# heliaxdev/ark-plonk

Measured on AMD Instinct MI355X. Metric: proofs/sec at 2^20 constraints (BLS12-381, KZG10); MSM G1-adds/s, higher is better.
Workload: dtype u32 limbs (256/384-bit Montgomery integers)

## Files before the change

### ark_plonk_amd/build.py

```python
from __future__ import annotations

import os
import subprocess
import sys
from concurrent.futures import ThreadPoolExecutor

HERE = os.path.dirname(os.path.abspath(__file__))
CSRC = os.path.join(HERE, "csrc")
OBJ = os.path.join(CSRC, "obj")
LIB = os.path.join(HERE, "libark_plonk_amd.so")
HIPCC = os.environ.get("HIPCC", "/opt/rocm/bin/hipcc")
FLAGS = ["--offload-arch=gfx950", "-O3", "-std=c++17", "-fPIC", "-Wall", "-Wno-unused-function", "-Wno-unused-variable",
         "-mllvm", "-pragma-unroll-threshold=1000000", "-Wpass-failed"]

FIELD_HDRS = ["field_common.cuh", "field.cuh", "fieldu.cuh", "fields.cuh", "curve_params.h", "zk_common.h"]
HOST_HDRS = FIELD_HDRS + ["ecu.cuh", "ctx.h", "g1_host.h", "../../include/ark_plonk_amd.h"]
API_HDRS = HOST_HDRS + ["api_internal.h"]
FR_IO, ZBOUND, POINT_IO = ["fr_io.cuh"], ["fr_io.cuh", "zbound.cuh"], ["point_io.cuh"]
DOMAIN, DEV_SCAN = ["fr_io.cuh", "domain.cuh"], ["dev_scan.cuh"]
GADGET = ["gadget_common.cuh"]
BLOCK_INV = ["block_inverse.cuh"]
G1_LIFT = ["g1_lift.cuh"]
PAIRING = ["pairing.cuh", "pairing_params.h"]
REPLAY = ["strobe.cuh", "replay_walk.cuh"]
API_UNITS = ("api_ctx", "residency", "srs", "commit", "round", "api_host", "api_poly")
MSM_UNITS = ("msm_accumulate", "msm_reduce", "msm_sort", "msm_plan")


def jobs():
    out = [(f"{u}.o", f"{u}.hip", [], API_HDRS + (DOMAIN if u == "api_poly" else [])) for u in API_UNITS] + [
        ("hostio.o", "hostio.hip", [], HOST_HDRS),
        ("wire.o", "wire.hip", [], HOST_HDRS + REPLAY),
        ("kzg.o", "kzg.hip", [], HOST_HDRS + ZBOUND),
        ("lookup.o", "lookup.hip", [], HOST_HDRS + ZBOUND + DEV_SCAN),
        ("grand_product.o", "grand_product.hip", [], HOST_HDRS + DOMAIN),
        ("quotient.o", "quotient.hip", [], HOST_HDRS + ZBOUND + DOMAIN),
        ("quadtest.o", "quadtest.hip", [], HOST_HDRS + ["ecq.cuh"]),
        ("ntt.o", "ntt.hip", [], HOST_HDRS + DOMAIN + ["ntt_pass.cuh"]),
        ("ntt_pass_table.o", "ntt_pass_table.hip", [], []),
        ("msm_dispatch.o", "msm_dispatch.hip", [], HOST_HDRS),
        ("ipa.o", "ipa.hip", [], API_HDRS + FR_IO + POINT_IO + BLOCK_INV),
        ("compile.o", "compile.hip", [], API_HDRS + DOMAIN + DEV_SCAN),
        ("check.o", "check.hip", [], API_HDRS + ZBOUND + DOMAIN),
        ("gadget_layout.o", "gadget_layout.hip", [], API_HDRS + FR_IO + GADGET),
        ("gadget_witness.o", "gadget_witness.hip", [], API_HDRS + FR_IO + GADGET + BLOCK_INV),
        ("lookup_map.o", "lookup_map.hip", [], API_HDRS + FR_IO),
        ("verify.o", "verify.hip", [], API_HDRS + DOMAIN + BLOCK_INV + G1_LIFT),
        ("replay.o", "replay.hip", [], API_HDRS + REPLAY),
        ("g1_segments.o", "g1_segments.hip", [], API_HDRS + BLOCK_INV),
        ("ipa_setup.o", "ipa_setup.hip", [], API_HDRS + BLOCK_INV + G1_LIFT + ["h2c.cuh"]),
        ("pairing.o", "pairing.hip", [], API_HDRS + PAIRING),
    ]
    for c in (0, 1):
        for unit in MSM_UNITS:
            out.append((f"{unit}_c{c}.o", f"{unit}.hip", [f"-DZK_CURVE_SEL={c}"] + os.environ.get("ARK_PLONK_AMD_MSM_FLAGS", "").split(),
                        HOST_HDRS + POINT_IO + ["msm_common.cuh"] + (["ecq.cuh"] if unit == "msm_reduce" else [])))
        for s in range(3, 10):
            out.append((f"ntt_pass_c{c}_s{s}.o", "ntt_pass_inst.hip", [f"-DZK_CURVE_SEL={c}", f"-DZK_NTT_S={s}"],
                        FIELD_HDRS + ["ntt_pass.cuh"]))
    return out


PMC_UNITS = {
    "pmc_msm_accumulate.json": [("msm_accumulate.hip", ["-DZK_CURVE_SEL=0"])],
    "pmc_ntt.json": [("ntt.hip", [])] + [("ntt_pass_inst.hip", ["-DZK_CURVE_SEL=0", f"-DZK_NTT_S={s}"]) for s in range(3, 10)],
}


def device_asm(src: str, defs=(), timeout: float = 900) -> str:
    import re
    cmd = [HIPCC] + FLAGS + list(defs) + ["--cuda-device-only", "-S", os.path.join(CSRC, src), "-o", "-"]
    r = subprocess.run(cmd, capture_output=True, text=True, timeout=timeout)
    if r.returncode != 0:
        raise RuntimeError("hipcc failed: " + " ".join(cmd) + "\n" + r.stderr[-4000:])
    return re.sub(r"__hip_cuid_[0-9a-f]+", "__hip_cuid_X", r.stdout)


def device_code_sha256(units, workers: int = 8) -> str:
    import hashlib
    with ThreadPoolExecutor(max_workers=workers) as ex:
        texts = list(ex.map(lambda u: device_asm(*u), units))
    return hashlib.sha256("".join(texts).encode()).hexdigest()


def _stale(target: str, deps) -> bool:
    if not os.path.exists(target):
        return True
    t = os.path.getmtime(target)
    return any(os.path.getmtime(d) > t for d in deps)


def build(force: bool = False, verbose: bool = False, workers: int | None = None) -> str:
    os.makedirs(OBJ, exist_ok=True)
    todo = []
    objs = []
    for obj, src, defs, hdrs in jobs():
        o = os.path.join(OBJ, obj)
        objs.append(o)
        deps = [os.path.join(CSRC, src)] + [os.path.join(CSRC, h) for h in hdrs]
        if force or _stale(o, deps):
            todo.append([HIPCC] + FLAGS + defs + ["-c", os.path.join(CSRC, src), "-o", o])
    todo.sort(key=lambda c: (0 if "/msm_" in " ".join(c[-3:]) else 1, -int(next((d.split("=")[1] for d in c if d.startswith("-DZK_NTT_S=")), 0))))

    def run(cmd):
        if verbose:
            print(" ".join(cmd), flush=True)
        r = subprocess.run(cmd, capture_output=True, text=True)
        if r.returncode != 0:
            raise RuntimeError("hipcc failed: " + " ".join(cmd) + "\n" + r.stderr[-4000:])
        return r.stderr

    if todo:
        n = workers or min(len(todo), max(1, (os.cpu_count() or 4)))
        with ThreadPoolExecutor(max_workers=n) as ex:
            for err in ex.map(run, todo):
                if verbose and err.strip():
                    print(err, file=sys.stderr)
    if force or todo or _stale(LIB, objs):
        cmd = [HIPCC, "--offload-arch=gfx950", "-shared", "-fPIC", "-o", LIB] + objs
        if verbose:
            print(" ".join(cmd[:6]), "...", flush=True)
        subprocess.check_call(cmd)
    return LIB


if __name__ == "__main__":
    print(build(force="--force" in sys.argv, verbose=True))
```

### ark_plonk_amd/csrc/fieldu.cuh

```cuda
#pragma once
#include "field_common.cuh"

template <class P>
struct Fu {
    static constexpr int NL = P::NL;
    static constexpr int SAT = P::SAT_WORDS;
    static constexpr uint32_t M = (1u << 29) - 1u;
    uint32_t v[NL];

    ZK_HD static Fu zero() {
        Fu r;
#pragma unroll
        for (int i = 0; i < NL; ++i) r.v[i] = 0;
        return r;
    }
    ZK_HD static Fu one() {
        Fu r;
#pragma unroll
        for (int i = 0; i < NL; ++i) r.v[i] = P::ONE(i);
        return r;
    }
    ZK_HD bool limbs_zero() const {
        uint32_t o = 0;
#pragma unroll
// ... 89 lines not shown
    }
    ZK_HD static Fu sub_raw8(const Fu& a, const Fu& b) {
        Fu t;
#pragma unroll
        for (int i = 0; i < NL; ++i) t.v[i] = a.v[i] + P::ZB8(i) - b.v[i];
        return t;
    }
    ZK_HD static Fu sub_raw16(const Fu& a, const Fu& b) {
        Fu t;
#pragma unroll
        for (int i = 0; i < NL; ++i) t.v[i] = a.v[i] + P::ZB16(i) - b.v[i];
        return t;
    }

    ZK_HD static Fu mul(const Fu& a, const Fu& b) {
        uint32_t m[NL];
        Fu r;
        uint64_t carry = 0;
#pragma unroll
        for (int k = 0; k < NL; ++k) {
            uint64_t a0 = 0, a1 = 0, am = 0;
#pragma unroll
            for (int i = 0; i <= k; ++i) {
                if (i & 1) a1 += (uint64_t)a.v[i] * b.v[k - i];
                else a0 += (uint64_t)a.v[i] * b.v[k - i];
            }
#pragma unroll
            for (int i = 0; i < k; ++i) am += (uint64_t)m[i] * P::MOD(k - i);
            uint64_t t = a0 + a1 + am + carry;
            m[k] = ((uint32_t)t * P::PINV) & M;
            t += (uint64_t)m[k] * P::MOD(0);
            carry = t >> 29;
        }
#pragma unroll
        for (int k = NL; k < 2 * NL - 1; ++k) {
            uint64_t a0 = 0, a1 = 0, am = 0;
#pragma unroll
            for (int i = k - NL + 1; i < NL; ++i) {
                if (i & 1) a1 += (uint64_t)a.v[i] * b.v[k - i];
                else a0 += (uint64_t)a.v[i] * b.v[k - i];
                am += (uint64_t)m[i] * P::MOD(k - i);
            }
            uint64_t t = a0 + a1 + am + carry;
            r.v[k - NL] = (uint32_t)t & M;
            carry = t >> 29;
        }
        r.v[NL - 1] = (uint32_t)carry;
        return r;
    }
    ZK_HD static uint64_t fence64(uint64_t t) {
#if defined(__HIP_DEVICE_COMPILE__)
        asm("" : "+v"(t));
#endif
        return t;
    }
    ZK_HD static Fu mul_fenced(const Fu& a, const Fu& b) {
        uint32_t m[NL];
        Fu r;
        uint64_t carry = 0;
#pragma unroll
        for (int k = 0; k < NL; ++k) {
            uint64_t t = fence64(carry + (uint64_t)a.v[0] * b.v[k]);
#pragma unroll
            for (int i = 1; i <= k; ++i) t += (uint64_t)a.v[i] * b.v[k - i];
#pragma unroll
            for (int i = 0; i < k; ++i) t += (uint64_t)m[i] * P::MOD(k - i);
            m[k] = ((uint32_t)t * P::PINV) & M;
            t += (uint64_t)m[k] * P::MOD(0);
            carry = t >> 29;
        }
#pragma unroll
        for (int k = NL; k < 2 * NL - 1; ++k) {
            uint64_t t = fence64(carry + (uint64_t)a.v[k - NL + 1] * b.v[NL - 1]);
#pragma unroll
            for (int i = k - NL + 2; i < NL; ++i) t += (uint64_t)a.v[i] * b.v[k - i];
#pragma unroll
            for (int i = k - NL + 1; i < NL; ++i) t += (uint64_t)m[i] * P::MOD(k - i);
            r.v[k - NL] = (uint32_t)t & M;
            carry = t >> 29;
        }
        r.v[NL - 1] = (uint32_t)carry;
        return r;
    }
    ZK_HD static Fu sqr(const Fu& a) {
        uint32_t m[NL], a2[NL];
        Fu r;
#pragma unroll
        for (int i = 0; i < NL; ++i) a2[i] = a.v[i] << 1;
        uint64_t carry = 0;
#pragma unroll
        for (int k = 0; k < NL; ++k) {
            uint64_t aa = 0, am = 0;
#pragma unroll
            for (int i = 0; 2 * i < k; ++i) aa += (uint64_t)a2[i] * a.v[k - i];
            if ((k & 1) == 0) aa += (uint64_t)a.v[k / 2] * a.v[k / 2];
#pragma unroll
            for (int i = 0; i < k; ++i) am += (uint64_t)m[i] * P::MOD(k - i);
            uint64_t t = aa + am + carry;
            m[k] = ((uint32_t)t * P::PINV) & M;
            t += (uint64_t)m[k] * P::MOD(0);
            carry = t >> 29;
        }
#pragma unroll
        for (int k = NL; k < 2 * NL - 1; ++k) {
            uint64_t aa = 0, am = 0;
#pragma unroll
            for (int i = k - NL + 1; 2 * i < k; ++i) aa += (uint64_t)a2[i] * a.v[k - i];
            if ((k & 1) == 0) aa += (uint64_t)a.v[k / 2] * a.v[k / 2];
#pragma unroll
            for (int i = k - NL + 1; i < NL; ++i) am += (uint64_t)m[i] * P::MOD(k - i);
            uint64_t t = aa + am + carry;
            r.v[k - NL] = (uint32_t)t & M;
            carry = t >> 29;
        }
        r.v[NL - 1] = (uint32_t)carry;
        return r;
    }

    ZK_HD bool is_zero_mod_reduced() const {
        if (v[0] != 0 && v[0] != P::MOD(0)) return false;
        uint32_t dz = 0, dp = 0;
#pragma unroll
        for (int i = 0; i < NL; ++i) {
            dz |= v[i];
            dp |= v[i] ^ P::MOD(i);
        }
        return dz == 0 || dp == 0;
    }
    ZK_HD bool is_zero_mod() const { return mul(*this, one()).is_zero_mod_reduced(); }

    ZK_HD static Fu canonical_lt2p(const Fu& a) {
        Fu d;
#pragma unroll
        for (int i = 0; i < NL; ++i) d.v[i] = a.v[i] - P::MOD(i);
        normalize(d);
        const bool neg = ((int32_t)d.v[NL - 1]) < 0;
        Fu r;
#pragma unroll
        for (int i = 0; i < NL; ++i) r.v[i] = neg ? a.v[i] : d.v[i];
        return r;
    }

    ZK_HD static Fu from_sat(const uint32_t* w) {
        Fu t = split_words(w);
        Fu c;
#pragma unroll
        for (int i = 0; i < NL; ++i) c.v[i] = P::C_IN(i);
        return mul(t, c);
    }
    ZK_HD void to_sat(uint32_t* w) const {
        Fu c;
#pragma unroll
        for (int i = 0; i < NL; ++i) c.v[i] = P::C_OUT(i);
        Fu t = canonical_lt2p(mul(*this, c));
        t.pack_words(w);
    }
    ZK_HD static Fu split_words(const uint32_t* w) {
        Fu t;
#pragma unroll
        for (int i = 0; i < NL; ++i) {
            const int bit = 29 * i;
            const int wi = bit >> 5, off = bit & 31;
            uint64_t lo = wi < SAT ? w[wi] : 0u;
            uint64_t hi = (wi + 1) < SAT ? w[wi + 1] : 0u;
            t.v[i] = (uint32_t)(((hi << 32) | lo) >> off) & M;
        }
// ... 16 lines not shown
```

### ark_plonk_amd/csrc/ntt.hip

```cpp
#include "ctx.h"
#include "domain.cuh"

#include "ntt_pass.cuh"

namespace {

template <class Fr>
struct PowBits {
    Fr p[32];
};
template <class Fr>
__global__ void gen_pow_table(void* out, uint64_t n, PowBits<Fr> pb, Fr mul, int mode, uint32_t log_m, uint32_t log_mprev, Fr to_rp) {
    uint64_t i = (uint64_t)blockIdx.x * blockDim.x + threadIdx.x;
    if (i >= n) return;
    uint64_t e = i;
    if (mode == 1) {
        uint64_t col = i & ((1ull << log_m) - 1);
        uint64_t k = i >> log_m;
        e = (col * k) & ((1ull << log_mprev) - 1);
    }
    Fr r = mul;
    for (int b = 0; b < 32; ++b) {
        if ((e >> b) & 1ull) r = Fr::mul(r, pb.p[b]);
    }
    st_fr<Fr>(out, i, Fr::mul(r, to_rp));
}

template <class FU>
__global__ void split_table(const void* packed, void* out, uint64_t n) {
    const uint64_t i = (uint64_t)blockIdx.x * blockDim.x + threadIdx.x;
    if (i >= n) return;
    const FU x = ld_u<FU>(packed, i);
    uint32_t w[4 * TW_INNER_U4];
#pragma unroll
    for (int k = 0; k < 4 * TW_INNER_U4; ++k) w[k] = k < FU::NL ? x.v[k] : 0u;
    uint4* q = reinterpret_cast<uint4*>(out) + TW_INNER_U4 * i;
#pragma unroll
    for (int k = 0; k < TW_INNER_U4; ++k) q[k] = make_uint4(w[4 * k], w[4 * k + 1], w[4 * k + 2], w[4 * k + 3]);
}

template <class Fr>
__global__ void ntt_tiny(const void* in, void* out, uint64_t in_len, uint32_t log_n, Fr w , Fr pre_g ,
                         Fr post_g , Fr scale ) {
    if (threadIdx.x != 0 || blockIdx.x != 0) return;
    const uint32_t n = 1u << log_n;
    Fr x[4], y[4];
    Fr gp = Fr::one();
    for (uint32_t i = 0; i < n; ++i) {
        x[i] = i < in_len ? Fr::mul(ld_fr<Fr>(in, i), gp) : Fr::zero();
        gp = Fr::mul(gp, pre_g);
    }
    Fr wi = Fr::one(), pg = scale;
    for (uint32_t i = 0; i < n; ++i) {
        Fr acc = Fr::zero(), wij = Fr::one();
        for (uint32_t j = 0; j < n; ++j) {
            acc = Fr::add(acc, Fr::mul(x[j], wij));
            wij = Fr::mul(wij, wi);
        }
        y[i] = Fr::mul(acc, pg);
        pg = Fr::mul(pg, post_g);
        wi = Fr::mul(wi, w);
    }
    for (uint32_t i = 0; i < n; ++i) st_fr<Fr>(out, i, y[i]);
}

template <class Fr>
__global__ void fr_convert_kernel(const void* in, void* out, uint64_t n, int to_mont) {
    uint64_t i = (uint64_t)blockIdx.x * blockDim.x + threadIdx.x;
    if (i >= n) return;
    Fr x = ld_fr<Fr>(in, i);
    st_fr<Fr>(out, i, to_mont ? Fr::to_mont(x) : Fr::from_mont(x));
}
template <class Fr>
__global__ void fr_mul_kernel(const void* a, const void* b, void* out, uint64_t n) {
    uint64_t i = (uint64_t)blockIdx.x * blockDim.x + threadIdx.x;
    if (i >= n) return;
    st_fr<Fr>(out, i, Fr::mul(ld_fr<Fr>(a, i), ld_fr<Fr>(b, i)));
}

template <class Fr>
PowBits<Fr> make_powbits(Fr base) {
    PowBits<Fr> pb;
    Fr cur = base;
    for (int b = 0; b < 32; ++b) {
        pb.p[b] = cur;
        cur = Fr::sqr(cur);
    }
    return pb;
}

template <class C>
int launch_pow_table(zk_ctx* c, void* out, uint64_t n, typename C::Fr base, typename C::Fr mul, int mode, uint32_t log_m,
                     uint32_t log_mprev) {
    typedef typename C::Fr Fr;
    if (n == 0) return ZK_OK;
    PowBits<Fr> pb = make_powbits(base);
    const Fr to_rp = to_rprime(Fr::one());
    const int T = 256;
    uint64_t blocks = (n + T - 1) / T;
    hipLaunchKernelGGL(gen_pow_table<Fr>, dim3((unsigned)blocks), dim3(T), 0, c->stream, out, n, pb, mul, mode, log_m, log_mprev, to_rp);
    ZK_HIP_TRY(hipGetLastError());
    return ZK_OK;
}

bool decompose(uint32_t log_n, int forced, int& n_pass, int s[4]) {
    s[0] = s[1] = s[2] = s[3] = 0;
    if (forced == 0 && log_n <= 9) {
        n_pass = 1;
        s[0] = (int)log_n;
        return true;
    }
    n_pass = forced ? forced : (int)((log_n + 8) / 9);
    if (n_pass > 4) return true;
    int base = (int)log_n / n_pass, extra = (int)log_n % n_pass;
    for (int i = 0; i < n_pass; ++i) s[i] = base + (i < extra ? 1 : 0);
    return forced == 0 || (s[n_pass - 1] >= 3 && s[0] <= 9);
}
int forced_passes(const zk_ctx* c, uint32_t log_n) { return log_n < 3 ? 0 : c->tune.ntt_passes; }

template <class C>
int get_inner_tw(zk_ctx* c, int s, bool inverse, void** out) {
    typedef typename C::Fr Fr;
    uint64_t key = ((uint64_t)C::ID << 40) | ((uint64_t)(inverse ? 1 : 0) << 32) | (uint64_t)s;
    auto it = c->inner_tw.find(key);
    if (it != c->inner_tw.end()) {
        *out = it->second;
        return ZK_OK;
    }
    uint64_t cnt = s >= 1 ? (1ull << (s - 1)) : 1;
    void* packed = nullptr;
    void* p = nullptr;
    if (hipMalloc(&packed, cnt * sizeof(Fr)) != hipSuccess) return zk_alloc_refused();
    if (hipMalloc(&p, cnt * TW_INNER_U4 * 16) != hipSuccess) {
        (void)hipFree(packed);
        return zk_alloc_refused();
    }
    Fr w = domain_root<C>((uint32_t)s);
    if (inverse) w = Fr::inverse(w);
    int rc = launch_pow_table<C>(c, packed, cnt, w, Fr::one(), 0, 0, 0);
    if (!rc) {
        const int T = 256;
        hipLaunchKernelGGL(split_table<typename C::FrU>, dim3((unsigned)((cnt + T - 1) / T)), dim3(T), 0, c->stream, packed, p, cnt);
        if (hipGetLastError() != hipSuccess || hipStreamSynchronize(c->stream) != hipSuccess) rc = ZK_ERR_HIP;
    }
    (void)hipFree(packed);
    if (rc) {
        (void)hipFree(p);
        return rc;
    }
    c->inner_tw[key] = p;
    *out = p;
    return ZK_OK;
}

template <class C>
int get_plan(zk_ctx* c, uint32_t log_n, bool inverse, NttPlan** out) {
    typedef typename C::Fr Fr;
    const int forced = forced_passes(c, log_n);
    uint64_t key = ((uint64_t)C::ID << 40) | ((uint64_t)forced << 36) | ((uint64_t)(inverse ? 1 : 0) << 32) | log_n;
    auto it = c->plans.find(key);
    if (it != c->plans.end()) {
        *out = it->second;
        return ZK_OK;
    }
    int n_pass, s[4];
    if (!decompose(log_n, forced, n_pass, s)) return ZK_ERR_UNSUPPORTED;
    NttPlan* pl = new NttPlan();
    pl->curve = C::ID;
    pl->log_n = log_n;
    pl->inverse = inverse;
    pl->n_pass = n_pass;
    for (int i = 0; i < 4; ++i) pl->s[i] = s[i];
    uint32_t log_mprev = log_n;
    for (int p = 0; p < pl->n_pass; ++p) {
        if (log_n >= 3) {
            int rc = get_inner_tw<C>(c, pl->s[p], inverse, &pl->tw_inner[p]);
            if (rc) { delete pl; return rc; }
        }
        if (p + 1 < pl->n_pass) {
            uint32_t log_m = log_mprev - (uint32_t)pl->s[p];
            uint64_t cnt = 1ull << log_mprev;
            hipError_t e = hipMalloc(&pl->tw_pass[p], cnt * sizeof(Fr));
            if (e != hipSuccess) { delete pl; return zk_alloc_refused(); }
            Fr w = domain_root<C>(log_mprev);
            if (inverse) w = Fr::inverse(w);
            int rc = launch_pow_table<C>(c, pl->tw_pass[p], cnt, w, Fr::one(), 1, log_m, log_mprev);
            if (rc) { delete pl; return rc; }
            log_mprev = log_m;
        }
    }
    c->plans[key] = pl;
    *out = pl;
    return ZK_OK;
}

template <class C>
int ensure_coset(zk_ctx* c, bool inv, uint64_t len, void** out) {
    typedef typename C::Fr Fr;
    DevBuf& buf = inv ? c->coset_inv_pow[C::ID] : c->coset_pow[C::ID];
    size_t& have = inv ? c->coset_inv_len[C::ID] : c->coset_len[C::ID];
    if (have < len) {
        ZK_HIP_TRY(hipStreamSynchronize(c->stream));
        uint64_t want = 1;
        while (want < len) want <<= 1;
        int rc = buf.ensure(want * sizeof(Fr));
        if (rc) return rc;
        Fr g = coset_gen<C>();
        if (inv) g = Fr::inverse(g);
        rc = launch_pow_table<C>(c, buf.p, want, g, Fr::one(), 0, 0, 0);
        if (rc) return rc;
        have = want;
    }
    *out = buf.p;
    return ZK_OK;
}

typedef int (*NttPassLauncher)(int final_pass, const NttPassArgs* a, hipStream_t st);
extern "C" NttPassLauncher zk_ntt_pass_launcher(int curve, int s);

template <class C>
int dispatch_pass(zk_ctx* c, int s, bool final_pass, const NttPassArgs& a) {
    if (s < 3 || s > 9) return ZK_ERR_UNSUPPORTED;
    NttPassLauncher fn = zk_ntt_pass_launcher(C::ID, s);
    if (!fn) return ZK_ERR_UNSUPPORTED;
    hipError_t e = (hipError_t)fn(final_pass ? 1 : 0, &a, c->stream);
    ZK_HIP_TRY(e);
    return ZK_OK;
}

template <class C>
int ntt_run(zk_ctx* c, int kind, uint32_t log_n, uint32_t n_polys, const void* const* d_ins, const size_t* in_lens, void* const* d_outs) {
    typedef typename C::Fr Fr;
    if (!domain_log_ok<C>(log_n)) return ZK_ERR_DOMAIN_TOO_LARGE;
    if (n_polys == 0 || n_polys > 16) return ZK_ERR_BAD_ARG;
    const uint64_t N = 1ull << log_n;
    size_t in_len = 0;
    bool all_quarter = true;
    for (uint32_t i = 0; i < n_polys; ++i) {
        if (in_lens[i] > N) return ZK_ERR_BAD_ARG;
        if (in_lens[i] > in_len) in_len = in_lens[i];
        if ((uint64_t)in_lens[i] * 4 > N) all_quarter = false;
    }
    const void* d_in = d_ins[0];
    void* d_out = d_outs[0];
    const bool inverse = (kind == ZK_NTT_IFFT || kind == ZK_NTT_COSET_IFFT);
    int rc;
    Fr n_inv = Fr::inverse(Fr::from_u64(N));
    if (log_n < 3) {
        Fr w = domain_root<C>(log_n);
        if (inverse) w = Fr::inverse(w);
        Fr g = coset_gen<C>();
        Fr pre_g = kind == ZK_NTT_COSET_FFT ? g : Fr::one();
        Fr post_g = kind == ZK_NTT_COSET_IFFT ? Fr::inverse(g) : Fr::one();
        ProfScope ps(c, "ntt_pass");
        for (uint32_t i = 0; i < n_polys; ++i)
            hipLaunchKernelGGL(ntt_tiny<Fr>, dim3(1), dim3(64), 0, c->stream, d_ins[i], d_outs[i], (uint64_t)in_lens[i], log_n, w, pre_g, post_g,
                               inverse ? n_inv : Fr::one());
        ZK_HIP_TRY(hipGetLastError());
        return ZK_OK;
    }
    {
        int np, sp[4];
        if (!decompose(log_n, forced_passes(c, log_n), np, sp)) return ZK_ERR_UNSUPPORTED;
    }
    void* pre = nullptr;
    void* post = nullptr;
    if (kind == ZK_NTT_COSET_FFT && in_len > 0) {
        rc = ensure_coset<C>(c, false, in_len, &pre);
        if (rc) return rc;
    }
    if (kind == ZK_NTT_COSET_IFFT) {
        rc = ensure_coset<C>(c, true, N, &post);
        if (rc) return rc;
    }
    NttPlan* pl = nullptr;
    rc = get_plan<C>(c, log_n, inverse, &pl);
    if (rc) return rc;
    if (pl->n_pass > 4) return ZK_ERR_UNSUPPORTED;
    void* work = nullptr;
    if (pl->n_pass > 1) {
        rc = c->ntt_work.ensure((size_t)n_polys * N * sizeof(Fr));
        if (rc) return rc;
        work = c->ntt_work.p;
    }
    uint32_t log_mprev = log_n;
    NttPassArgs a;
    ProfScope ps(c, "ntt_pass");
    for (int p = 0; p < pl->n_pass; ++p) {
        const int s = pl->s[p];
        const bool last = (p + 1 == pl->n_pass);
        memset(&a, 0, sizeof a);
        a.log_n = log_n;
        a.in = (p == 0) ? d_in : work;
        a.out = last ? d_out : work;
        a.in_len = (p == 0) ? in_lens[0] : N;
        if (n_polys > 1) {
            a.n_batch = n_polys;
            for (uint32_t i = 0; i < n_polys; ++i) {
                void* wk = (char*)work + (size_t)i * N * sizeof(Fr);
                a.ins[i] = (p == 0) ? d_ins[i] : wk;
                a.outs[i] = last ? d_outs[i] : wk;
                a.in_lens[i] = (p == 0) ? in_lens[i] : N;
            }
        }
        a.tw_inner = pl->tw_inner[p];
        a.pre_mul = (p == 0) ? pre : nullptr;
        const uint32_t LC = 9u - (uint32_t)s;
        if (!last) {
            uint32_t log_m = log_mprev - (uint32_t)s;
            uint32_t logc = LC < log_m ? LC : log_m;
            a.logc = logc;
            a.log_m = log_m;
            a.log_mprev = log_mprev;
            a.tw_pass = pl->tw_pass[p];
            a.n_tiles = (uint32_t)(N >> ((uint32_t)s + logc));
            a.quarter = (p == 0 && s >= 3 && all_quarter) ? 1u : 0u;
            log_mprev = log_m;
        } else {
            uint32_t s1 = (pl->n_pass > 1) ? (uint32_t)pl->s[0] : 0;
            uint32_t logc = LC < s1 ? LC : s1;
            a.logc = logc;
            a.s1 = s1;
            a.s2 = pl->n_pass == 4 ? (uint32_t)pl->s[1] : 0u;
            a.post_mul = post;
            const Fr sc = to_rprime(inverse ? n_inv : Fr::one());
            for (int i = 0; i < 8; ++i) a.scale[i] = sc.v[i];
            a.n_tiles = (uint32_t)(N >> ((uint32_t)s + logc));
        }
        rc = dispatch_pass<C>(c, s, last, a);
        if (rc) return rc;
        if (c->profiling) c->prof["ntt_passes"].launches += 1;
    }
    return ZK_OK;
}

}

int ntt_run_dev(zk_ctx* c, int curve, int kind, uint32_t log_n, const void* d_in, size_t in_len, void* d_out) {
    return ntt_run_batch_dev(c, curve, kind, log_n, 1, &d_in, &in_len, &d_out);
}

int ntt_run_batch_dev(zk_ctx* c, int curve, int kind, uint32_t log_n, uint32_t n_polys, const void* const* d_ins, const size_t* in_lens,
                      void* const* d_outs) {
    if (kind < 0 || kind > 3) return ZK_ERR_BAD_ARG;
    for (uint32_t base = 0; base < n_polys; base += 16) {
        const uint32_t cnt = n_polys - base < 16 ? n_polys - base : 16;
        const int rc = zk_on_curve(curve, ZK_ERR_BAD_ARG, [&](auto cv) {
            return ntt_run<decltype(cv)>(c, kind, log_n, cnt, d_ins + base, in_lens + base, d_outs + base);
        });
        if (rc) return rc;
    }
    return ZK_OK;
}

int ntt_prepare(zk_ctx* c, int curve, uint32_t log_n) {
    NttPlan* pl;
    if (log_n < 3) return ZK_OK;
    for (int inv = 0; inv < 2; ++inv) {
        const int rc = zk_on_curve(curve, ZK_ERR_BAD_ARG, [&](auto cv) {
            typedef decltype(cv) Cv;
            if (!domain_log_ok<Cv>(log_n)) return ZK_ERR_DOMAIN_TOO_LARGE;
            return get_plan<Cv>(c, log_n, inv != 0, &pl);
        });
        if (rc) return rc;
    }
    return ZK_OK;
}

void ntt_ctx_free(zk_ctx* c) {
    for (auto& kv : c->plans) delete kv.second;
    c->plans.clear();
    for (auto& kv : c->inner_tw) (void)hipFree(kv.second);
    c->inner_tw.clear();
    c->ntt_work.release();
    for (int i = 0; i < 2; ++i) {
        c->coset_pow[i].release();
        c->coset_inv_pow[i].release();
    }
}

static int fr_convert_on(int curve, int to_mont, const void* d_in, size_t n, void* d_out, hipStream_t st) {
    if (n == 0) return ZK_OK;
    const int T = 256;
    unsigned blocks = (unsigned)((n + T - 1) / T);
    const int rc = zk_on_curve(curve, ZK_ERR_BAD_ARG, [&](auto cv) {
        hipLaunchKernelGGL(fr_convert_kernel<typename decltype(cv)::Fr>, dim3(blocks), dim3(T), 0, st, d_in, d_out, (uint64_t)n, to_mont);
        return ZK_OK;
    });
    if (rc) return rc;
    ZK_HIP_TRY(hipGetLastError());
    return ZK_OK;
}
int fr_convert_dev(zk_ctx* c, int curve, int to_mont, const void* d_in, size_t n, void* d_out) {
    return fr_convert_on(curve, to_mont, d_in, n, d_out, c->stream);
}
int fr_convert_stream(zk_ctx* c, int curve, const void* d_in, size_t n, void* d_out, hipStream_t st) {
    (void)c;
// ... 16 lines not shown
```

### ark_plonk_amd/csrc/ntt_pass.cuh

```cuda
#pragma once
#include <hip/hip_runtime.h>
#include "curve_params.h"
#include "field.cuh"
#include "fieldu.cuh"

typedef __attribute__((address_space(3))) volatile uint32_t lds_u32;

struct NttPassArgs {
    const void* in;
    void* out;
    const void* tw_inner;
    const void* tw_pass;
    const void* pre_mul;
    const void* post_mul;
    uint32_t scale[8];
    uint64_t in_len;
    uint32_t log_n;
    uint32_t logc;
    uint32_t log_m;
    uint32_t log_mprev;
    uint32_t s1;
    uint32_t s2;
    uint32_t n_tiles;
    uint32_t quarter;
    uint32_t n_batch;
    const void* ins[16];
    void* outs[16];
    uint64_t in_lens[16];
};

__host__ __device__ inline uint32_t bitrev32(uint32_t x, int bits) {
#if defined(__HIP_DEVICE_COMPILE__)
    return bits ? __brev(x) >> (32 - bits) : 0u;
#else
    uint32_t r = 0;
    for (int i = 0; i < bits; ++i) { r = (r << 1) | (x & 1); x >>= 1; }
    return r;
#endif
}

template <class F>
ZK_D F ld_u(const void* base, uint64_t idx) {
    const uint4* q = reinterpret_cast<const uint4*>(base) + 2 * idx;
    uint4 a = q[0], b = q[1];
    uint32_t w[8] = {a.x, a.y, a.z, a.w, b.x, b.y, b.z, b.w};
    return F::split_words(w);
}
template <class F>
ZK_D void st_u(void* base, uint64_t idx, const F& x) {
    uint32_t w[8];
    F::canonical_lt2p(x).pack_words(w);
    uint4* q = reinterpret_cast<uint4*>(base) + 2 * idx;
    q[0] = make_uint4(w[0], w[1], w[2], w[3]);
    q[1] = make_uint4(w[4], w[5], w[6], w[7]);
}

template <class F>
ZK_D void st_u_raw(void* base, uint64_t idx, const F& x) {
    uint32_t w[8];
    x.pack_words(w);
    uint4* q = reinterpret_cast<uint4*>(base) + 2 * idx;
    q[0] = make_uint4(w[0], w[1], w[2], w[3]);
    q[1] = make_uint4(w[4], w[5], w[6], w[7]);
}

constexpr int TW_INNER_U4 = 3;
template <class F>
ZK_D F ld_limbs(const void* base, uint64_t idx) {
    static_assert(F::NL <= 4 * TW_INNER_U4, "inner twiddle entry too small");
    const uint4* q = reinterpret_cast<const uint4*>(base) + TW_INNER_U4 * idx;
    F r;
#pragma unroll
    for (int i = 0; i < TW_INNER_U4; ++i) {
        if (4 * i >= F::NL) break;
        const uint4 a = q[i];
        if (4 * i + 0 < F::NL) r.v[4 * i + 0] = a.x;
        if (4 * i + 1 < F::NL) r.v[4 * i + 1] = a.y;
        if (4 * i + 2 < F::NL) r.v[4 * i + 2] = a.z;
        if (4 * i + 3 < F::NL) r.v[4 * i + 3] = a.w;
    }
    return r;
}

constexpr int ntt_units_before(int t) {
    int b = 1;
    for (int s = 0; s < t; ++s) {
        if (b > 6) b = 1;
        b += 2;
    }
    return b;
}
constexpr bool ntt_sweep_at(int t) { return ntt_units_before(t) > 6; }
static_assert(ntt_units_before(1) == 3 && ntt_units_before(2) == 5 && ntt_units_before(3) == 7 && ntt_units_before(4) == 3, "two units per stage");
static_assert(!ntt_sweep_at(0) && !ntt_sweep_at(2) && ntt_sweep_at(3) && !ntt_sweep_at(5) && ntt_sweep_at(6) && ntt_sweep_at(9), "a sweep every third stage");

template <int B0>
ZK_D uint32_t window_pos(uint32_t v, uint32_t e) {
    return ((v >> B0) << (B0 + 3)) | (e << B0) | (v & ((1u << B0) - 1u));
}

template <class F>
ZK_D void wave_exchange(F (&x)[8], lds_u32* sc, const uint32_t (&widx)[8], const uint32_t (&ridx)[8]) {
#pragma unroll
    for (int l = 0; l < F::NL; ++l) {
#pragma unroll
        for (int e = 0; e < 8; ++e) sc[widx[e]] = x[e].v[l];
        __builtin_amdgcn_wave_barrier();
#pragma unroll
        for (int e = 0; e < 8; ++e) x[e].v[l] = sc[ridx[e]];
        __builtin_amdgcn_wave_barrier();
    }
}

template <class F, int S, int B0, int LB_LO, int LB_HI>
ZK_D void dit_window(F (&x)[8], uint32_t v, const void* tw, bool quarter) {
    const uint32_t vlow = v & ((1u << B0) - 1u);
#pragma unroll
    for (int lb = LB_LO; lb < LB_HI; ++lb) {
        const int t = B0 + lb;
        if (ntt_sweep_at(t)) {
#pragma unroll
            for (int e = 0; e < 8; ++e) F::sweep(x[e]);
        }
#pragma unroll
        for (int e = 0; e < 8; ++e) {
            if (e & (1 << lb)) continue;
            const int eo = e | (1 << lb);
            if constexpr (B0 == 0 && LB_LO == 0) {
                if (lb < 2 && quarter) {
                    x[eo] = x[e];
                    continue;
                }
                if (lb == 0) {
                    const F b = x[eo];
                    x[eo] = F::sub_raw3(x[e], b);
                    x[e] = F::add_raw(x[e], b);
                    continue;
                }
                if ((e & ((1 << lb) - 1)) == 0) {
                    F b = x[eo];
                    F::sweep(b);
                    x[eo] = lb == 1 ? F::sub_raw8(x[e], b) : F::sub_raw16(x[e], b);
                    x[e] = F::add_raw(x[e], b);
                    continue;
                }
            }
            const uint32_t plow = ((uint32_t)(e & ((1 << lb) - 1)) << B0) | vlow;
            const uint32_t j = plow << (S - 1 - t);
            F w = ld_limbs<F>(tw, j);
            F m = F::mul_fenced(x[eo], w);
            x[eo] = F::sub_raw3(x[e], m);
            x[e] = F::add_raw(x[e], m);
        }
    }
}

template <class F, int S, int B0>
ZK_D void dit_all(F (&x)[8], uint32_t v, uint32_t c, uint32_t LC, const void* tw, lds_u32* sc, bool quarter = false) {
    constexpr int REM = S - B0;
    if constexpr (REM >= 3) {
        dit_window<F, S, B0, 0, 3>(x, v, tw, quarter);
        if constexpr (REM > 3) {
            constexpr int NB0 = (REM - 3 >= 3) ? B0 + 3 : S - 3;
            uint32_t wi[8], ri[8];
#pragma unroll
            for (int e = 0; e < 8; ++e) {
                wi[e] = (window_pos<B0>(v, e) << LC) | c;
                ri[e] = (window_pos<NB0>(v, e) << LC) | c;
            }
            wave_exchange<F>(x, sc, wi, ri);
            if constexpr (REM - 3 >= 3) {
                dit_all<F, S, B0 + 3>(x, v, c, LC, tw, sc);
            } else {
                dit_window<F, S, S - 3, 3 - (REM - 3), 3>(x, v, tw, false);
            }
        }
    }
}

template <class F, int S>
__global__ void __launch_bounds__(256) ntt_pass_mid(NttPassArgs a) {
    constexpr uint32_t LC = 9 - S;
    __shared__ uint32_t scratch[4][512];
    const uint32_t lane = threadIdx.x & 63, wv = threadIdx.x >> 6;
    const uint32_t tile = blockIdx.x * (blockDim.x >> 6) + wv;
    if (tile >= a.n_tiles) return;
    const void* in = a.in;
    void* out = a.out;
    uint64_t in_len = a.in_len;
    if (a.n_batch) {
        in = a.ins[blockIdx.y];
        out = a.outs[blockIdx.y];
        in_len = a.in_lens[blockIdx.y];
    }
    lds_u32* sc = (lds_u32*)scratch[wv];
    const uint32_t c = lane & ((1u << LC) - 1u);
    const uint32_t v = lane >> LC;
    const bool active = c < (1u << a.logc);
    const uint32_t lcg = a.log_m - a.logc;
    const uint64_t blk = (uint64_t)tile >> lcg;
    const uint64_t cg = (uint64_t)tile & ((1ull << lcg) - 1);
    const uint64_t col = (cg << a.logc) + c;
    const uint64_t base = (blk << a.log_mprev) + col;

    F x[8];
#pragma unroll
    for (int e = 0; e < 8; ++e) {
        const uint64_t row = bitrev32((v << 3) | e, S);
        const uint64_t idx = base + (row << a.log_m);
        if (active && idx < in_len) {
            x[e] = ld_u<F>(in, idx);
            if (a.pre_mul) x[e] = F::mul_fenced(x[e], ld_u<F>(a.pre_mul, idx));
        } else {
            x[e] = F::zero();
        }
    }
    dit_all<F, S, 0>(x, v, c, LC, a.tw_inner, sc, a.quarter != 0);
    if (!active) return;
#pragma unroll
    for (int e = 0; e < 8; ++e) {
        const uint64_t k = S >= 3 ? (((uint64_t)e << (S - 3)) | v) : e;
        F w = ld_u<F>(a.tw_pass, (k << a.log_m) + col);
        if (ntt_units_before(S) > 6) F::sweep(x[e]);
        st_u_raw<F>(out, base + (k << a.log_m), F::mul_fenced(x[e], w));
    }
}

template <class F, int S>
__global__ void __launch_bounds__(256) ntt_pass_final(NttPassArgs a) {
    constexpr uint32_t L = 1u << S;
    constexpr uint32_t LC = 9 - S;
    __shared__ uint32_t scratch[4][512];
    const uint32_t lane = threadIdx.x & 63, wv = threadIdx.x >> 6;
    const uint32_t tile = blockIdx.x * (blockDim.x >> 6) + wv;
    if (tile >= a.n_tiles) return;
    const void* in = a.in;
    void* out = a.out;
    uint64_t in_len = a.in_len;
    if (a.n_batch) {
        in = a.ins[blockIdx.y];
        out = a.outs[blockIdx.y];
        in_len = a.in_lens[blockIdx.y];
    }
    lds_u32* sc = (lds_u32*)scratch[wv];
    const uint32_t log_nb = a.log_n - S;
    const uint32_t log_rest = log_nb - a.s1;
    const uint32_t lg = a.s1 - a.logc;
    const uint64_t rho = (uint64_t)tile >> lg;
    const uint64_t g = (uint64_t)tile & ((1ull << lg) - 1);

    F x[8];
    uint32_t wi[8], ri[8];
    const uint32_t c = lane & ((1u << LC) - 1u);
    const uint32_t v = lane >> LC;
#pragma unroll
    for (int e = 0; e < 8; ++e) {
        const uint32_t q = (uint32_t)e * 64u + lane;
        const uint32_t cb = q >> S, row = q & (L - 1);
        const uint64_t b = ((((uint64_t)g << a.logc) + cb) << log_rest) | rho;
        const uint64_t idx = (b << S) + row;
        if (cb < (1u << a.logc) && idx < in_len) {
            x[e] = ld_u<F>(in, idx);
            if (a.pre_mul) x[e] = F::mul_fenced(x[e], ld_u<F>(a.pre_mul, idx));
        } else {
            x[e] = F::zero();
        }
        wi[e] = (bitrev32(row, S) << LC) | cb;
        ri[e] = (((v << 3) | (uint32_t)e) << LC) | c;
    }
    wave_exchange<F>(x, sc, wi, ri);
    dit_all<F, S, 0>(x, v, c, LC, a.tw_inner, sc);
    if (c >= (1u << a.logc)) return;
    const uint64_t k1o = ((uint64_t)g << a.logc) + c;
    uint64_t rho_rev = rho;
    if (a.s2) {
        const uint32_t s3 = log_rest - a.s2;
        rho_rev = (rho >> s3) | ((rho & ((1ull << s3) - 1ull)) << a.s2);
    }
    const uint64_t obase = k1o + (rho_rev << a.s1);
    F sc_mul = F::split_words(a.scale);
#pragma unroll
    for (int e = 0; e < 8; ++e) {
        const uint64_t k = S >= 3 ? (((uint64_t)e << (S - 3)) | v) : e;
        const uint64_t oidx = obase + (k << log_nb);
        if (ntt_units_before(S) > 6) F::sweep(x[e]);
        F y = F::mul_fenced(x[e], sc_mul);
        if (a.post_mul) y = F::mul_fenced(y, ld_u<F>(a.post_mul, oidx));
        st_u<F>(out, oidx, y);
    }
}
```

### ark_plonk_amd/csrc/ntt_pass_inst.hip

```cpp
#include "ntt_pass.cuh"

#if ZK_CURVE_SEL == 0
typedef Fu<FrBls12_381UParams> FrSel;
#define ZK_LAUNCHER_NAME2(s) zk_ntt_pass_c0_s##s
#else
typedef Fu<FrBn254UParams> FrSel;
#define ZK_LAUNCHER_NAME2(s) zk_ntt_pass_c1_s##s
#endif
#define ZK_LAUNCHER_NAME(s) ZK_LAUNCHER_NAME2(s)

extern "C" int ZK_LAUNCHER_NAME(ZK_NTT_S)(int final_pass, const NttPassArgs* a, hipStream_t st) {
    constexpr int S = ZK_NTT_S;
    const unsigned waves = a->n_tiles < 4 ? a->n_tiles : 4;
    const unsigned blocks = (a->n_tiles + waves - 1) / waves;
    const unsigned polys = a->n_batch ? a->n_batch : 1;
    if (final_pass)
        hipLaunchKernelGGL((ntt_pass_final<FrSel, S>), dim3(blocks, polys), dim3(64 * waves), 0, st, *a);
    else
        hipLaunchKernelGGL((ntt_pass_mid<FrSel, S>), dim3(blocks, polys), dim3(64 * waves), 0, st, *a);
    return (int)hipGetLastError();
}
```

Measured before the change: 13.08.

## Store NTT twiddle and coset tables as pre-split limbs and specialize pass kernels

Twiddle, pass-twiddle (when small) and pre/post-multiplier tables are now generated directly in 29-bit limb layout, which removes the separate split_table pass and the per-load unpacking in the NTT kernels. Pass kernels are specialized at compile time on whether a pre-multiplier exists and whether twiddles come as limbs. Branchy input loads are replaced with clamped unconditional loads plus zero masking. A new mul_chain variant with asm register fences forces a serial accumulation order. The quarter shortcut is split into separate paths. Limb-format tables take more memory than packed ones, and the extra kernel variants grow code size.

```diff
diff --git a/ark_plonk_amd/build.py b/ark_plonk_amd/build.py
--- a/ark_plonk_amd/build.py
+++ b/ark_plonk_amd/build.py
@@ -57,7 +57,7 @@
                         HOST_HDRS + POINT_IO + ["msm_common.cuh"] + (["ecq.cuh"] if unit == "msm_reduce" else [])))
         for s in range(3, 10):
             out.append((f"ntt_pass_c{c}_s{s}.o", "ntt_pass_inst.hip", [f"-DZK_CURVE_SEL={c}", f"-DZK_NTT_S={s}"],
-                        FIELD_HDRS + ["ntt_pass.cuh"]))
+                        FIELD_HDRS + ["ecu.cuh", "ntt_pass.cuh"]))
     return out
 
 
diff --git a/ark_plonk_amd/csrc/fieldu.cuh b/ark_plonk_amd/csrc/fieldu.cuh
--- a/ark_plonk_amd/csrc/fieldu.cuh
+++ b/ark_plonk_amd/csrc/fieldu.cuh
@@ -195,6 +195,41 @@
         r.v[NL - 1] = (uint32_t)carry;
         return r;
     }
+    ZK_HD static uint64_t link(uint64_t t) {
+#if defined(__HIP_DEVICE_COMPILE__)
+        asm volatile("" : : "v"(t));
+#endif
+        return t;
+    }
+    ZK_HD static Fu mul_chain(const Fu& a, const Fu& b) {
+        uint32_t m[NL];
+        Fu r;
+        uint64_t carry = 0;
+#pragma unroll
+        for (int k = 0; k < NL; ++k) {
+            uint64_t t = (uint64_t)a.v[0] * b.v[k];
+            if (k) t = link(carry + t);
+#pragma unroll
+            for (int i = 1; i <= k; ++i) t = link(t + (uint64_t)a.v[i] * b.v[k - i]);
+#pragma unroll
+            for (int i = 0; i < k; ++i) t = link(t + (uint64_t)m[i] * P::MOD(k - i));
+            m[k] = ((uint32_t)t * P::PINV) & M;
+            t += (uint64_t)m[k] * P::MOD(0);
+            carry = t >> 29;
+        }
+#pragma unroll
+        for (int k = NL; k < 2 * NL - 1; ++k) {
+            uint64_t t = link(carry + (uint64_t)a.v[k - NL + 1] * b.v[NL - 1]);
+#pragma unroll
+            for (int i = k - NL + 2; i < NL; ++i) t = link(t + (uint64_t)a.v[i] * b.v[k - i]);
+#pragma unroll
+            for (int i = k - NL + 1; i < NL; ++i) t = link(t + (uint64_t)m[i] * P::MOD(k - i));
+            r.v[k - NL] = (uint32_t)t & M;
+            carry = t >> 29;
+        }
+        r.v[NL - 1] = (uint32_t)carry;
+        return r;
+    }
     ZK_HD static Fu sqr(const Fu& a) {
         uint32_t m[NL], a2[NL];
         Fu r;
diff --git a/ark_plonk_amd/csrc/ntt.hip b/ark_plonk_amd/csrc/ntt.hip
--- a/ark_plonk_amd/csrc/ntt.hip
+++ b/ark_plonk_amd/csrc/ntt.hip
@@ -9,8 +9,8 @@
 struct PowBits {
     Fr p[32];
 };
-template <class Fr>
-__global__ void gen_pow_table(void* out, uint64_t n, PowBits<Fr> pb, Fr mul, int mode, uint32_t log_m, uint32_t log_mprev, Fr to_rp) {
+template <class Fr, class FU>
+__global__ void gen_pow_table(void* out, uint64_t n, PowBits<Fr> pb, Fr mul, int mode, uint32_t log_m, uint32_t log_mprev, Fr to_rp, int limbs) {
     uint64_t i = (uint64_t)blockIdx.x * blockDim.x + threadIdx.x;
     if (i >= n) return;
     uint64_t e = i;
@@ -23,20 +23,9 @@
     for (int b = 0; b < 32; ++b) {
         if ((e >> b) & 1ull) r = Fr::mul(r, pb.p[b]);
     }
-    st_fr<Fr>(out, i, Fr::mul(r, to_rp));
-}
-
-template <class FU>
-__global__ void split_table(const void* packed, void* out, uint64_t n) {
-    const uint64_t i = (uint64_t)blockIdx.x * blockDim.x + threadIdx.x;
-    if (i >= n) return;
-    const FU x = ld_u<FU>(packed, i);
-    uint32_t w[4 * TW_INNER_U4];
-#pragma unroll
-    for (int k = 0; k < 4 * TW_INNER_U4; ++k) w[k] = k < FU::NL ? x.v[k] : 0u;
-    uint4* q = reinterpret_cast<uint4*>(out) + TW_INNER_U4 * i;
-#pragma unroll
-    for (int k = 0; k < TW_INNER_U4; ++k) q[k] = make_uint4(w[4 * k], w[4 * k + 1], w[4 * k + 2], w[4 * k + 3]);
+    const Fr y = Fr::mul(r, to_rp);
+    if (limbs) st_limbs<FU>(out, i, FU::split_words(y.v));
+    else st_fr<Fr>(out, i, y);
 }
 
 template <class Fr>
@@ -78,6 +67,9 @@
     st_fr<Fr>(out, i, Fr::mul(ld_fr<Fr>(a, i), ld_fr<Fr>(b, i)));
 }
 
+constexpr size_t TABLE_ENTRY_BYTES = TW_INNER_U4 * 16;
+constexpr bool tw_pass_in_limbs(uint32_t log_mprev) { return log_mprev <= 20; }
+
 template <class Fr>
 PowBits<Fr> make_powbits(Fr base) {
     PowBits<Fr> pb;
@@ -91,14 +83,15 @@
 
 template <class C>
 int launch_pow_table(zk_ctx* c, void* out, uint64_t n, typename C::Fr base, typename C::Fr mul, int mode, uint32_t log_m,
-                     uint32_t log_mprev) {
+                     uint32_t log_mprev, bool limbs = true) {
     typedef typename C::Fr Fr;
     if (n == 0) return ZK_OK;
     PowBits<Fr> pb = make_powbits(base);
     const Fr to_rp = to_rprime(Fr::one());
     const int T = 256;
     uint64_t blocks = (n + T - 1) / T;
-    hipLaunchKernelGGL(gen_pow_table<Fr>, dim3((unsigned)blocks), dim3(T), 0, c->stream, out, n, pb, mul, mode, log_m, log_mprev, to_rp);
+    hipLaunchKernelGGL((gen_pow_table<Fr, typename C::FrU>), dim3((unsigned)blocks), dim3(T), 0, c->stream, out, n, pb, mul, mode, log_m, log_mprev, to_rp,
+                       limbs ? 1 : 0);
     ZK_HIP_TRY(hipGetLastError());
     return ZK_OK;
 }
@@ -128,22 +121,11 @@
         return ZK_OK;
     }
     uint64_t cnt = s >= 1 ? (1ull << (s - 1)) : 1;
-    void* packed = nullptr;
     void* p = nullptr;
-    if (hipMalloc(&packed, cnt * sizeof(Fr)) != hipSuccess) return zk_alloc_refused();
-    if (hipMalloc(&p, cnt * TW_INNER_U4 * 16) != hipSuccess) {
-        (void)hipFree(packed);
-        return zk_alloc_refused();
-    }
+    if (hipMalloc(&p, cnt * TABLE_ENTRY_BYTES) != hipSuccess) return zk_alloc_refused();
     Fr w = domain_root<C>((uint32_t)s);
     if (inverse) w = Fr::inverse(w);
-    int rc = launch_pow_table<C>(c, packed, cnt, w, Fr::one(), 0, 0, 0);
-    if (!rc) {
-        const int T = 256;
-        hipLaunchKernelGGL(split_table<typename C::FrU>, dim3((unsigned)((cnt + T - 1) / T)), dim3(T), 0, c->stream, packed, p, cnt);
-        if (hipGetLastError() != hipSuccess || hipStreamSynchronize(c->stream) != hipSuccess) rc = ZK_ERR_HIP;
-    }
-    (void)hipFree(packed);
+    int rc = launch_pow_table<C>(c, p, cnt, w, Fr::one(), 0, 0, 0);
     if (rc) {
         (void)hipFree(p);
         return rc;
@@ -180,11 +162,12 @@
         if (p + 1 < pl->n_pass) {
             uint32_t log_m = log_mprev - (uint32_t)pl->s[p];
             uint64_t cnt = 1ull << log_mprev;
-            hipError_t e = hipMalloc(&pl->tw_pass[p], cnt * sizeof(Fr));
+            const bool limbs = tw_pass_in_limbs(log_mprev);
+            hipError_t e = hipMalloc(&pl->tw_pass[p], cnt * (limbs ? TABLE_ENTRY_BYTES : sizeof(Fr)));
             if (e != hipSuccess) { delete pl; return zk_alloc_refused(); }
             Fr w = domain_root<C>(log_mprev);
             if (inverse) w = Fr::inverse(w);
-            int rc = launch_pow_table<C>(c, pl->tw_pass[p], cnt, w, Fr::one(), 1, log_m, log_mprev);
+            int rc = launch_pow_table<C>(c, pl->tw_pass[p], cnt, w, Fr::one(), 1, log_m, log_mprev, limbs);
             if (rc) { delete pl; return rc; }
             log_mprev = log_m;
         }
@@ -203,7 +186,7 @@
         ZK_HIP_TRY(hipStreamSynchronize(c->stream));
         uint64_t want = 1;
         while (want < len) want <<= 1;
-        int rc = buf.ensure(want * sizeof(Fr));
+        int rc = buf.ensure(want * TABLE_ENTRY_BYTES);
         if (rc) return rc;
         Fr g = coset_gen<C>();
         if (inv) g = Fr::inverse(g);
@@ -313,6 +296,7 @@
             a.log_m = log_m;
             a.log_mprev = log_mprev;
             a.tw_pass = pl->tw_pass[p];
+            a.tw_limbs = tw_pass_in_limbs(log_mprev) ? 1u : 0u;
             a.n_tiles = (uint32_t)(N >> ((uint32_t)s + logc));
             a.quarter = (p == 0 && s >= 3 && all_quarter) ? 1u : 0u;
             log_mprev = log_m;
diff --git a/ark_plonk_amd/csrc/ntt_pass.cuh b/ark_plonk_amd/csrc/ntt_pass.cuh
--- a/ark_plonk_amd/csrc/ntt_pass.cuh
+++ b/ark_plonk_amd/csrc/ntt_pass.cuh
@@ -3,6 +3,7 @@
 #include "curve_params.h"
 #include "field.cuh"
 #include "fieldu.cuh"
+#include "ecu.cuh"
 
 typedef __attribute__((address_space(3))) volatile uint32_t lds_u32;
 
@@ -23,6 +24,7 @@
     uint32_t s2;
     uint32_t n_tiles;
     uint32_t quarter;
+    uint32_t tw_limbs;
     uint32_t n_batch;
     const void* ins[16];
     void* outs[16];
@@ -47,6 +49,14 @@
     return F::split_words(w);
 }
 template <class F>
+ZK_D F ld_u_or_zero(const void* base, uint64_t idx, bool keep) {
+    const uint4* q = reinterpret_cast<const uint4*>(base) + 2 * idx;
+    uint4 a = q[0], b = q[1];
+    uint32_t w[8] = {keep ? a.x : 0u, keep ? a.y : 0u, keep ? a.z : 0u, keep ? a.w : 0u,
+                     keep ? b.x : 0u, keep ? b.y : 0u, keep ? b.z : 0u, keep ? b.w : 0u};
+    return F::split_words(w);
+}
+template <class F>
 ZK_D void st_u(void* base, uint64_t idx, const F& x) {
     uint32_t w[8];
     F::canonical_lt2p(x).pack_words(w);
@@ -81,6 +91,15 @@
     }
     return r;
 }
+template <class F>
+ZK_D void st_limbs(void* base, uint64_t idx, const F& x) {
+    uint32_t w[4 * TW_INNER_U4];
+#pragma unroll
+    for (int k = 0; k < 4 * TW_INNER_U4; ++k) w[k] = k < F::NL ? x.v[k] : 0u;
+    uint4* q = reinterpret_cast<uint4*>(base) + TW_INNER_U4 * idx;
+#pragma unroll
+    for (int k = 0; k < TW_INNER_U4; ++k) q[k] = make_uint4(w[4 * k], w[4 * k + 1], w[4 * k + 2], w[4 * k + 3]);
+}
 
 constexpr int ntt_units_before(int t) {
     int b = 1;
@@ -112,54 +131,65 @@
     }
 }
 
-template <class F, int S, int B0, int LB_LO, int LB_HI>
+template <class F, int S, int B0>
+ZK_D void dit_stage(F (&x)[8], uint32_t vlow, const void* tw, int lb) {
+    const int t = B0 + lb;
+    if (ntt_sweep_at(t)) {
+#pragma unroll
+        for (int e = 0; e < 8; ++e) F::sweep(x[e]);
+    }
+#pragma unroll
+    for (int e = 0; e < 8; ++e) {
+        if (e & (1 << lb)) continue;
+        const int eo = e | (1 << lb);
+        if constexpr (B0 == 0) {
+            if (lb == 0) {
+                const F b = x[eo];
+                x[eo] = F::sub_raw3(x[e], b);
+                x[e] = F::add_raw(x[e], b);
+                continue;
+            }
+            if ((e & ((1 << lb) - 1)) == 0) {
+                F b = x[eo];
+                F::sweep(b);
+                x[eo] = lb == 1 ? F::sub_raw8(x[e], b) : F::sub_raw16(x[e], b);
+                x[e] = F::add_raw(x[e], b);
+                continue;
+            }
+        }
+        const uint32_t plow = ((uint32_t)(e & ((1 << lb) - 1)) << B0) | vlow;
+        const uint32_t j = plow << (S - 1 - t);
+        F w = ld_limbs<F>(tw, j);
+        F m = F::mul_chain(x[eo], w);
+        x[eo] = F::sub_raw3(x[e], m);
+        x[e] = F::add_raw(x[e], m);
+    }
+}
+template <class F, int S, int B0, int LB_LO, int LB_HI, bool Q>
 ZK_D void dit_window(F (&x)[8], uint32_t v, const void* tw, bool quarter) {
     const uint32_t vlow = v & ((1u << B0) - 1u);
-#pragma unroll
-    for (int lb = LB_LO; lb < LB_HI; ++lb) {
-        const int t = B0 + lb;
-        if (ntt_sweep_at(t)) {
-#pragma unroll
-            for (int e = 0; e < 8; ++e) F::sweep(x[e]);
-        }
-#pragma unroll
-        for (int e = 0; e < 8; ++e) {
-            if (e & (1 << lb)) continue;
-            const int eo = e | (1 << lb);
-            if constexpr (B0 == 0 && LB_LO == 0) {
-                if (lb < 2 && quarter) {
-                    x[eo] = x[e];
-                    continue;
-                }
-                if (lb == 0) {
-                    const F b = x[eo];
-                    x[eo] = F::sub_raw3(x[e], b);
-                    x[e] = F::add_raw(x[e], b);
-                    continue;
-                }
-                if ((e & ((1 << lb) - 1)) == 0) {
-                    F b = x[eo];
-                    F::sweep(b);
-                    x[eo] = lb == 1 ? F::sub_raw8(x[e], b) : F::sub_raw16(x[e], b);
-                    x[e] = F::add_raw(x[e], b);
-                    continue;
-                }
-            }
-            const uint32_t plow = ((uint32_t)(e & ((1 << lb) - 1)) << B0) | vlow;
-            const uint32_t j = plow << (S - 1 - t);
-            F w = ld_limbs<F>(tw, j);
-            F m = F::mul_fenced(x[eo], w);
-            x[eo] = F::sub_raw3(x[e], m);
-            x[e] = F::add_raw(x[e], m);
-        }
-    }
-}
-
-template <class F, int S, int B0>
+    if constexpr (Q && B0 == 0 && LB_LO == 0 && LB_HI >= 2) {
+        if (zk_apart(quarter)) {
+            x[1] = x[2] = x[3] = x[0];
+            x[5] = x[6] = x[7] = x[4];
+        }
+        if (zk_apart(!quarter)) {
+            dit_stage<F, S, B0>(x, vlow, tw, 0);
+            dit_stage<F, S, B0>(x, vlow, tw, 1);
+        }
+#pragma unroll
+        for (int lb = 2; lb < LB_HI; ++lb) dit_stage<F, S, B0>(x, vlow, tw, lb);
+    } else {
+#pragma unroll
+        for (int lb = LB_LO; lb < LB_HI; ++lb) dit_stage<F, S, B0>(x, vlow, tw, lb);
+    }
+}
+
+template <class F, int S, int B0, bool Q = false>
 ZK_D void dit_all(F (&x)[8], uint32_t v, uint32_t c, uint32_t LC, const void* tw, lds_u32* sc, bool quarter = false) {
     constexpr int REM = S - B0;
     if constexpr (REM >= 3) {
-        dit_window<F, S, B0, 0, 3>(x, v, tw, quarter);
+        dit_window<F, S, B0, 0, 3, Q>(x, v, tw, quarter);
         if constexpr (REM > 3) {
             constexpr int NB0 = (REM - 3 >= 3) ? B0 + 3 : S - 3;
             uint32_t wi[8], ri[8];
@@ -172,13 +202,13 @@
             if constexpr (REM - 3 >= 3) {
                 dit_all<F, S, B0 + 3>(x, v, c, LC, tw, sc);
             } else {
-                dit_window<F, S, S - 3, 3 - (REM - 3), 3>(x, v, tw, false);
+                dit_window<F, S, S - 3, 3 - (REM - 3), 3, false>(x, v, tw, false);
             }
         }
     }
 }
 
-template <class F, int S>
+template <class F, int S, bool PRE, bool TWL>
 __global__ void __launch_bounds__(256) ntt_pass_mid(NttPassArgs a) {
     constexpr uint32_t LC = 9 - S;
     __shared__ uint32_t scratch[4][512];
@@ -203,30 +233,34 @@
     const uint64_t col = (cg << a.logc) + c;
     const uint64_t base = (blk << a.log_mprev) + col;
 
+    const void* src = in_len ? in : a.tw_inner;
+    const uint64_t last = in_len ? in_len - 1 : 0;
     F x[8];
 #pragma unroll
     for (int e = 0; e < 8; ++e) {
         const uint64_t row = bitrev32((v << 3) | e, S);
         const uint64_t idx = base + (row << a.log_m);
-        if (active && idx < in_len) {
-            x[e] = ld_u<F>(in, idx);
-            if (a.pre_mul) x[e] = F::mul_fenced(x[e], ld_u<F>(a.pre_mul, idx));
-        } else {
-            x[e] = F::zero();
-        }
-    }
-    dit_all<F, S, 0>(x, v, c, LC, a.tw_inner, sc, a.quarter != 0);
+        const uint64_t at = idx < in_len ? idx : last;
+        const bool keep = active && idx < in_len;
+        x[e] = ld_u_or_zero<F>(src, at, keep);
+        if constexpr (PRE) {
+            if (zk_apart(keep)) x[e] = F::mul_chain(x[e], ld_limbs<F>(a.pre_mul, at));
+        }
+    }
+    dit_all<F, S, 0, true>(x, v, c, LC, a.tw_inner, sc, a.quarter != 0);
     if (!active) return;
 #pragma unroll
     for (int e = 0; e < 8; ++e) {
         const uint64_t k = S >= 3 ? (((uint64_t)e << (S - 3)) | v) : e;
-        F w = ld_u<F>(a.tw_pass, (k << a.log_m) + col);
+        F w;
+        if constexpr (TWL) w = ld_limbs<F>(a.tw_pass, (k << a.log_m) + col);
+        else w = ld_u<F>(a.tw_pass, (k << a.log_m) + col);
         if (ntt_units_before(S) > 6) F::sweep(x[e]);
-        st_u_raw<F>(out, base + (k << a.log_m), F::mul_fenced(x[e], w));
-    }
-}
-
-template <class F, int S>
+        st_u_raw<F>(out, base + (k << a.log_m), F::mul_chain(x[e], w));
+    }
+}
+
+template <class F, int S, bool PRE>
 __global__ void __launch_bounds__(256) ntt_pass_final(NttPassArgs a) {
     constexpr uint32_t L = 1u << S;
     constexpr uint32_t LC = 9 - S;
@@ -249,6 +283,8 @@
     const uint64_t rho = (uint64_t)tile >> lg;
     const uint64_t g = (uint64_t)tile & ((1ull << lg) - 1);
 
+    const void* src = in_len ? in : a.tw_inner;
+    const uint64_t last = in_len ? in_len - 1 : 0;
     F x[8];
     uint32_t wi[8], ri[8];
     const uint32_t c = lane & ((1u << LC) - 1u);
@@ -259,11 +295,11 @@
         const uint32_t cb = q >> S, row = q & (L - 1);
         const uint64_t b = ((((uint64_t)g << a.logc) + cb) << log_rest) | rho;
         const uint64_t idx = (b << S) + row;
-        if (cb < (1u << a.logc) && idx < in_len) {
-            x[e] = ld_u<F>(in, idx);
-            if (a.pre_mul) x[e] = F::mul_fenced(x[e], ld_u<F>(a.pre_mul, idx));
-        } else {
-            x[e] = F::zero();
+        const uint64_t at = idx < in_len ? idx : last;
+        const bool keep = cb < (1u << a.logc) && idx < in_len;
+        x[e] = ld_u_or_zero<F>(src, at, keep);
+        if constexpr (PRE) {
+            if (zk_apart(keep)) x[e] = F::mul_chain(x[e], ld_limbs<F>(a.pre_mul, at));
         }
         wi[e] = (bitrev32(row, S) << LC) | cb;
         ri[e] = (((v << 3) | (uint32_t)e) << LC) | c;
@@ -280,12 +316,14 @@
     const uint64_t obase = k1o + (rho_rev << a.s1);
     F sc_mul = F::split_words(a.scale);
 #pragma unroll
+    for (int i = 0; i < F::NL; ++i) asm("" : "+v"(sc_mul.v[i]));
+#pragma unroll
     for (int e = 0; e < 8; ++e) {
         const uint64_t k = S >= 3 ? (((uint64_t)e << (S - 3)) | v) : e;
         const uint64_t oidx = obase + (k << log_nb);
         if (ntt_units_before(S) > 6) F::sweep(x[e]);
-        F y = F::mul_fenced(x[e], sc_mul);
-        if (a.post_mul) y = F::mul_fenced(y, ld_u<F>(a.post_mul, oidx));
+        F y = F::mul_chain(x[e], sc_mul);
+        if (a.post_mul) y = F::mul_chain(y, ld_limbs<F>(a.post_mul, oidx));
         st_u<F>(out, oidx, y);
     }
 }
diff --git a/ark_plonk_amd/csrc/ntt_pass_inst.hip b/ark_plonk_amd/csrc/ntt_pass_inst.hip
--- a/ark_plonk_amd/csrc/ntt_pass_inst.hip
+++ b/ark_plonk_amd/csrc/ntt_pass_inst.hip
@@ -14,9 +14,10 @@
     const unsigned waves = a->n_tiles < 4 ? a->n_tiles : 4;
     const unsigned blocks = (a->n_tiles + waves - 1) / waves;
     const unsigned polys = a->n_batch ? a->n_batch : 1;
-    if (final_pass)
-        hipLaunchKernelGGL((ntt_pass_final<FrSel, S>), dim3(blocks, polys), dim3(64 * waves), 0, st, *a);
-    else
-        hipLaunchKernelGGL((ntt_pass_mid<FrSel, S>), dim3(blocks, polys), dim3(64 * waves), 0, st, *a);
+    void (*kernel)(NttPassArgs);
+    if (final_pass) kernel = a->pre_mul ? ntt_pass_final<FrSel, S, true> : ntt_pass_final<FrSel, S, false>;
+    else if (a->tw_limbs) kernel = a->pre_mul ? ntt_pass_mid<FrSel, S, true, true> : ntt_pass_mid<FrSel, S, false, true>;
+    else kernel = a->pre_mul ? ntt_pass_mid<FrSel, S, true, false> : ntt_pass_mid<FrSel, S, false, false>;
+    hipLaunchKernelGGL(kernel, dim3(blocks, polys), dim3(64 * waves), 0, st, *a);
     return (int)hipGetLastError();
 }
```

After: 13.16 (median of 6 runs). About the same (+0.6%).
